# Lymphatus/caesium-clt

Hardware: AMD Instinct MI355X
Metric: megapixels/sec JPEG q=80 1920x1080 batch (higher is better)
Workload: dtype int32

## Files before the change

caesium-clt_amd/binding.py:

```python
import ctypes as C
import os

_HERE = os.path.dirname(os.path.abspath(__file__))
NPHASES = 8
NKERNELS = 36
PHASE_NAMES = ["decode", "pixel", "masks_flags_runs", "stats_tables", "sizes_scan", "pack", "stuff_assemble", "reserved"]


class CCSParameters(C.Structure):
    _fields_ = [("keep_metadata", C.c_bool), ("jpeg_quality", C.c_uint32), ("jpeg_chroma_subsampling", C.c_uint32),
                ("jpeg_progressive", C.c_bool), ("jpeg_optimize", C.c_bool), ("jpeg_preserve_icc", C.c_bool),
                ("png_quality", C.c_uint32), ("png_optimization_level", C.c_uint32), ("png_force_zopfli", C.c_bool),
                ("png_optimize", C.c_bool), ("gif_quality", C.c_uint32), ("webp_quality", C.c_uint32), ("webp_lossless", C.c_bool),
                ("tiff_compression", C.c_uint32), ("tiff_deflate_level", C.c_uint32), ("width", C.c_uint32), ("height", C.c_uint32)]


class CCSResult(C.Structure):
    _fields_ = [("success", C.c_bool), ("code", C.c_uint32), ("error_message", C.c_char_p)]


class CByteArray(C.Structure):
    _fields_ = [("data", C.POINTER(C.c_uint8)), ("length", C.c_size_t)]


class Timing(C.Structure):
    _fields_ = [("total_ms", C.c_float), ("phase_ms", C.c_float * NPHASES), ("kernel_ms", C.c_float * NKERNELS), ("in_bytes", C.c_uint64), ("out_bytes", C.c_uint64),
                ("pixels", C.c_uint64), ("coef_bytes", C.c_uint64), ("n_images", C.c_uint32), ("n_failed", C.c_uint32), ("n_seq_decoded", C.c_uint32), ("n_par_fallback", C.c_uint32), ("n_par_short", C.c_uint32), ("n_prog_decoded", C.c_uint32), ("n_refine_chains", C.c_uint32), ("n_search_extra", C.c_uint32), ("n_fused_lists", C.c_uint32), ("n_list_refine", C.c_uint32), ("n_ac_in_lists", C.c_uint32), ("n_list_runs", C.c_uint32)]


class PngTiming(C.Structure):
    _fields_ = [("total_ms", C.c_float), ("kernel_ms", C.c_float * 16), ("in_bytes", C.c_uint64), ("out_bytes", C.c_uint64), ("pixels", C.c_uint64),
                ("raw_bytes", C.c_uint64), ("n_images", C.c_uint32), ("n_failed", C.c_uint32), ("n_trials", C.c_uint32)]


class CaesiumError(RuntimeError):
    def __init__(self, code, message):
        super().__init__(f"[{code}] {message}")
        self.code = code


def library_path():
    return os.path.join(_HERE, "libcaesium_hip.so")
# ... 412 lines not shown
```

caesium-clt_amd/csrc/batch.hpp:

```cpp
#pragma once
#include <array>
#include <chrono>
#include <map>
#include <string>
#include <vector>

#include "../../include/caesium_hip.h"
#include "devmem.hpp"
#include "jpeg_host.hpp"
#include "kernels.h"
#include "webp_kernels.h"

namespace csh {

struct Item {
    int code = 0;
    std::string msg;
    JpegInfo in;
    JpegInfo out;
    int image = -1;
    size_t file_size = 0;
    std::vector<uint8_t> meta_out;
};

// ... 59 lines not shown
    int cand_work[64]; int ncand;
    int Al_luma = 0, Al_chroma = 0;
    uint64_t best_luma = 0, best_chroma = 0;
    int split_luma = 0, split_chroma = 0;
    bool luma_on = false, chroma_on = false;
};

struct EncodePlan {
    std::vector<EncScan> script;
    std::vector<ScanWork> swork;
    uint32_t nslots = 0, nlist_slots = 0, ntok_slots = 0;
    uint32_t nref_slots = 0;
    uint32_t last_run_refine = 0;
    uint32_t list_run = CSH_LIST_RUN;
    uint32_t nlist_runs = 0, nref_runs = 0;
    uint32_t last_run_list_runs = 0;
    uint64_t total_corr = 0;
    uint64_t total_units = 0, total_words = 0;
    uint32_t max_units = 0;
    int ntables = 0;
    std::vector<TokPlan> plans;
    std::vector<int> plan_comp, plan_image;
    std::vector<EChunk> echunks;
    uint64_t tok_cap = 0;
    uint32_t tok_scale = 1;
    std::vector<TokRegion> regions;
    std::vector<uint32_t> region_est;
    uint32_t hist_rows = 0;
    std::vector<NzList> nzlists;
    std::vector<NzSet> nzsets;
// ... 152 lines not shown
    for (int i = 0; i < int(sizeof kKernelSlots / sizeof kKernelSlots[0]); i++) if (kKernelSlots[i].slot != i) return false;
    return true;
}
static_assert(sizeof kKernelSlots / sizeof kKernelSlots[0] == CSH_NKERNELS && int(KS_COUNT) == int(CSH_NKERNELS), "one row per csh_timing.kernel_ms slot");
static_assert(kernel_slots_in_order(), "row i of kKernelSlots describes slot i");

struct PlanSwitches {
    std::string profile;
    bool nz_once = true;
    bool tr_sort = true;
    int prog_par = -1;
    bool fused_420 = true;
    bool nz_fused = true;
    bool ref_list = true;
    uint32_t list_run = CSH_LIST_RUN;
    bool ac_tiles = false;
    static PlanSwitches read();
};

struct Laps {
    const bool trace;
    std::chrono::steady_clock::time_point at = std::chrono::steady_clock::now();
    std::string text;
    Laps();
    void lap(const char *what);
};

struct BatchPlanner {
    csh_batch *const b;
    const CByteArray *const inputs;
// ... 53 lines not shown
```

caesium-clt_amd/csrc/batch_plan.cpp:

```cpp
#include <algorithm>
#include <atomic>
#include <cmath>
#include <thread>

#include "batch.hpp"
#include "resize_host.h"

namespace csh {

static void build_dev_huff(const HuffSpec &h, DevHuff &d) {
    memset(&d, 0, sizeof d);
    for (int l = 0; l < 18; l++) d.maxcode[l] = -1;
    if (!h.present) return;
    int code = 0, p = 0;
    for (int l = 1; l <= 16; l++) {
        if (h.bits[l]) {
            d.valptr[l] = p - code;
            for (int i = 0; i < h.bits[l]; i++, p++, code++)
                if (l <= 9) {
                    int base = code << (9 - l);
                    for (int k = 0; k < (1 << (9 - l)); k++) d.look[(base + k) & 511] = uint16_t((l << 8) | h.vals[p]);
                }
            d.maxcode[l] = code - 1;
        }
// ... 179 lines not shown
        b->enc.nzlists[i].base = at; b->enc.nzlists[i].cap = uint32_t(cap);
        at += (cap + 3) & ~uint64_t(3);
    }
    b->enc.nz_cap = at + 64;
}

PlanSwitches PlanSwitches::read() {
    auto is = [](const char *name, const char *v) { const char *e = getenv(name); return e && !strcmp(e, v); };
    PlanSwitches s;
    const char *penv = getenv("CSH_PROFILE");
    s.profile = penv && *penv ? penv : "mozjpeg";
    s.nz_once = !is("CSH_NZ_ONCE", "0");
    s.tr_sort = !is("CSH_TR_SORT", "0");
    s.nz_fused = !is("CSH_NZ_FUSED", "0");
    s.ac_tiles = is("CSH_AC_TILES", "1");
    s.ref_list = is("CSH_REF_LIST", "1") || (s.ref_list && !is("CSH_REF_LIST", "0"));
    const char *pp = getenv("CSH_PROG_PAR");
    s.prog_par = pp && !strcmp(pp, "0") ? 0 : (pp && !strcmp(pp, "1") ? 1 : -1);
    s.fused_420 = !getenv("CSH_NO_FUSED_420");
    if (const char *lr = getenv("CSH_LIST_RUN")) { if (*lr) s.list_run = uint32_t(std::min(32, std::max(1, atoi(lr)))); }
    return s;
}

Laps::Laps() : trace(getenv("CSH_TRACE") != nullptr) {}
void Laps::lap(const char *what) {
    if (!trace) return;
    const auto now = std::chrono::steady_clock::now();
    char buf[64];
    snprintf(buf, sizeof buf, " %s %.1f", what, std::chrono::duration<double, std::milli>(now - at).count());
    text += buf; at = now;
}

BatchPlanner::BatchPlanner(csh_batch *b_, const CByteArray *inputs_, size_t count_, const CCSParameters *p_, const csp_pixels *px_)
    : b(b_), inputs(inputs_), count(count_), p(p_), px(px_), sw(PlanSwitches::read()), progressive(p_->jpeg_progressive) {}

void BatchPlanner::begin() {
    b->items.resize(count);
    quality_table(int(p->jpeg_quality), qout_nat);
    DevQuant qo; make_quant(qout_nat, qo);
    b->quants.push_back(qo);
    b->q_base = int(b->quants.size()) - 1;
    for (int q = 1; q <= 100; q++) { uint16_t tq[64]; quality_table(q, tq); DevQuant dq; make_quant(tq, dq); b->quants.push_back(dq); }
    b->progressive = progressive;
    b->enc.list_run = sw.list_run;

    add_script(b->enc.script, 3, true);
    add_script(b->enc.script, 1, true);
    add_script(b->enc.script, 3, false);
    add_script(b->enc.script, 1, false);
    script_base3 = progressive ? 0 : 16; script_base1 = progressive ? 10 : 17;
    const bool webp = b->webp, rgb_out = b->rgb_out;
    const std::string &profile = sw.profile;
    b->enc.search = progressive && !webp && !rgb_out && profile != "plain";
    const bool lossy_jpeg = !b->lossless && !webp && !rgb_out;
    b->tr.trellis = lossy_jpeg && (profile == "mozjpeg" || profile == "mozjpeg-trellis");
    b->tr.dering = lossy_jpeg && (profile == "mozjpeg" || profile == "mozjpeg-dering");
    b->tr.nz_once = b->tr.trellis && progressive && sw.nz_once && sw.tr_sort;
}

// ... 842 lines not shown
```

caesium-clt_amd/csrc/batch_run.cpp:

```cpp
#include <algorithm>

#include "batch.hpp"

namespace csh {
namespace {

class KernelMarks {
    hipEvent_t ev[CSH_NKERNELS + 1];
    int created = 0, next = 0;
    const hipStream_t st;

public:
    explicit KernelMarks(hipStream_t s) : st(s) {}
    KernelMarks(const KernelMarks &) = delete;
    KernelMarks &operator=(const KernelMarks &) = delete;
    ~KernelMarks() { for (int i = 0; i < created; i++) (void)hipEventDestroy(ev[i]); }
    int start() {
        for (; created <= CSH_NKERNELS; created++) CSH_CHECK(hipEventCreate(&ev[created]));
        CSH_CHECK(hipEventRecord(ev[0], st));
        return 0;
    }
    int claim(KernelSlot slot, hipEvent_t *e) {
        if (int(slot) != next || next >= CSH_NKERNELS) {
            csh_set_error("internal: timing mark '%s' out of order (slot %d is next)", slot < KS_COUNT ? kKernelSlots[slot].name : "?", next);
// ... 217 lines not shown

    int encode_begin() {
        fill_enc_ctx();
        launch_reset_works(st, b->enc.d_swork.p, c.nwork);
        if (!fused && (b->enc.d_nz_cursor.zero(st) || b->enc.d_nz_chunk_cnt.zero(st))) return -1;
        if (b->enc.d_symbits.zero(st) || b->enc.d_eobbits.zero(st) || (!eobrun_cleared && b->enc.d_eobrun.zero(st)) || b->enc.d_tables.zero(st) || b->enc.d_tok_cursor.zero(st) || b->enc.d_slot_eobh.zero(st) || b->enc.d_scan_pad.zero(st)) return -1;
#ifdef CSH_EMUL
        if (b->enc.d_raw.zero(st)) return -1;
#else
        if ((c.debug & 8192u) && b->enc.d_raw.zero(st)) return -1;
#endif
        MARK(KS_MEMSET_ENC);
        return 0;
    }

    void count_list_runs(const Stage &sg, bool gate) {
        for (uint32_t wi = sg.work0; (sg.nlr || sg.nrr) && wi < sg.work0 + sg.nwork; wi++) {
            const ScanWork &w = b->enc.swork[wi];
            if ((w.lr_base != 0xFFFFFFFFu || w.rr_base != 0xFFFFFFFFu) && (!gate || b->enc.work_active[wi])) b->enc.last_run_list_runs += ((w.nunits + 255u) / 256u + b->enc.list_run - 1u) / b->enc.list_run;
        }
    }

    void set_stage(const Stage &sg) {
        c.echunks = b->enc.d_echunks.p + sg.ech0; c.nechunks = sg.nech; c.slot0 = sg.slot0; c.nslots = sg.nslots;
        c.nzchunks = (fused ? b->enc.d_nzchunks_fused.p : b->enc.d_nzchunks.p) + sg.nzc0; c.nnzchunks = sg.nnzc;
        c.nz_build = sg.nz_build[fused ? 1 : 0]; c.nz_filter = sg.nz_filter[fused ? 1 : 0];
        c.list_slots = b->enc.d_list_slots.p + sg.ls0; c.nlist_slots = sg.nls; c.tok_slots = b->enc.d_tok_slots.p + sg.ts0; c.ntok_slots = sg.nts;
        c.ref_slots = b->enc.d_ref_slots.p + sg.rs0; c.nref_slots = sg.nrs;
        c.list_runs = b->enc.d_list_runs.p + sg.lr0; c.nlist_runs = sg.nlr; c.ref_runs = b->enc.d_ref_runs.p + sg.rr0; c.nref_runs = sg.nrr; c.list_run = b->enc.list_run;
    }

    int trellis() {
        const Stage &tg = b->tr.tstage;
        set_stage(tg);
        c.stats_only = 1;
        if (b->enc.d_long_cnt.zero(st)) return -1;
        c.nz_blk_cnt = b->tr.t_sort ? b->tr.d_tblk_cnt.p : nullptr;
        c.nz_blk_off = (b->tr.t_sort && b->tr.nz_once) ? b->tr.d_tblk_off.p : nullptr;
        launch_nzlist(st, c);
        c.nz_blk_cnt = nullptr; c.nz_blk_off = nullptr;
        if (b->tr.t_sort) {
            TrellisCtx ts;
            memset(&ts, 0, sizeof ts);
            ts.work = b->tr.d_twork.p; ts.nwork = int(b->tr.twork.size()); ts.blk_cnt = b->tr.d_tblk_cnt.p; ts.perm = b->tr.d_tperm.p;
            launch_trellis_sort(st, ts);
        }
        launch_tokens(st, c);
        launch_list_stats(st, c);
        count_list_runs(tg, false);
        launch_ac_runs(st, c);
        launch_gen_tables(st, b->enc.d_tables.p + tg.table0, int(tg.ntables));
        c.stats_only = 0;
        if (b->enc.d_nz_cursor.zero(st)) return -1;
        MARK(KS_TRELLIS_STATS);
        TrellisCtx tc;
        fill_trellis_ctx(tc);
        if (b->tr.d_tqueue.zero(st)) return -1;
        launch_trellis_ac(st, tc);
        MARK(KS_TRELLIS_AC);
        launch_trellis_dc(st, tc);
        launch_fix_dummy(st, b->d_imgs.p, nimg, b->max_dummy, b->d_coef.p);
        MARK(KS_TRELLIS_DC);
        return 0;
    }

    int stage(const Stage &sg, bool mark, bool gate) {
#define SMARK(slot) do { if (mark) MARK(slot); } while (0)
        set_stage(sg);
        c.work_active = gate ? b->enc.d_work_active.p : nullptr;
        a.work0 = int(sg.work0); a.nwork_run = int(sg.nwork);
        if (b->enc.d_long_cnt.zero(st)) return -1;
        launch_nzlist(st, c);
        SMARK(KS_NZLIST);
        launch_list_refine(st, c);
        for (uint32_t wi = sg.work0; sg.nrs && wi < sg.work0 + sg.nwork; wi++)
            if (b->enc.swork[wi].rs_base != 0xFFFFFFFFu && (!gate || b->enc.work_active[wi])) b->enc.last_run_refine++;
        count_list_runs(sg, gate);
        launch_tokens(st, c);
        SMARK(KS_TOKENS);
        launch_list_stats(st, c);
        SMARK(KS_LIST_STATS);
        launch_ac_runs(st, c);
        SMARK(KS_AC_RUNS);
        launch_gen_tables(st, b->enc.d_tables.p + sg.table0, int(sg.ntables));
        SMARK(KS_GEN_TABLES);
        launch_chunk_sizes(st, c);
        SMARK(KS_CHUNK_SIZES);
        launch_exclusive_scan(st, b->enc.d_chunk_bits.p + sg.slot0, b->enc.d_chunk_off.p + sg.slot0, sg.nslots, b->enc.d_scan_tmp.p, b->enc.d_scan_tmp.n);
        SMARK(KS_SCAN_CHUNK_BITS);
        launch_scan_sizes(st, a);
        launch_exclusive_scan(st, b->enc.d_scan_pad.p, b->enc.d_scan_raw_off.p, uint64_t(a.nwork), b->enc.d_scan_tmp.p, b->enc.d_scan_tmp.n);
        launch_scan_place(st, a);
// ... 72 lines not shown
        if (b->out.d_img_size.zero(st)) return -1;
        csw::launch_webp_yuv(st, b->wp.d_wimgs.p, nwimg, b->wp.wmax_luma, b->pix.d_rgb.p, b->wp.d_wwork.p);
        MARK(KS_WEBP_YUV);
        hipEvent_t mid;
        if (marks.claim(KS_WEBP_ENCODE, &mid)) return -1;
        if (csw::launch_webp_encode(st, b->wp.wimgs.data(), nwimg, b->wp.d_wimgs.p, b->wp.d_wwork.p, b->wp.d_wlevels.p, b->wp.d_wscratch.p, b->wp.d_wpart.p, b->out.d_out.p, b->out.d_img_size.p, b->out.d_status.p, mid)) return -1;
        MARK(KS_WEBP_ASSEMBLE);
        return finish(false);
    }
};

}

int run_once(csh_batch *b, csh_timing *t, bool requant_only) {
    Run r(b, t);
    b->enc.last_run_list_runs = 0;
    b->enc.last_run_fused = 0; b->enc.last_run_refine = 0; b->enc.last_run_ac_lists = 0;
    if (r.pools() || r.marks.start()) return -1;
    const bool from_pixels = requant_only && b->tr.dering;
    if (requant_only && !from_pixels) {
        if (r.requant()) return -1;
    } else {
        if (from_pixels ? r.skip_decode() : r.decode()) return -1;
        if (r.planes()) return -1;
        if (b->webp) return r.webp();
        if (b->rgb_out) return (r.marks.mark(KS_XFORM_DIRECT) || r.finish(false)) ? -1 : 0;
        if (r.pixels()) return -1;
    }
    if (r.encode_begin()) return -1;
    b->enc.last_run_fused = r.fused ? b->enc.n_fused : 0u;
    b->enc.last_run_ac_lists = r.fused ? b->enc.n_ac_lists : 0u;
// ... 9 lines not shown
```

caesium-clt_amd/csrc/k_aclist.hip:

```cpp
#include "kernels.h"
#include "wave.h"

namespace csh {

#define CSH_LP_WORDS 1024

__device__ __forceinline__ static uint32_t lbitlen(uint32_t v) { return 32u - uint32_t(__clz(v)); }
__device__ __forceinline__ static int lwave() { return int(threadIdx.x) / CSP_WAVE_THREADS; }

#define CSH_NZ_HALF 16
__device__ __forceinline__ static uint4 nz_load(const EncCtx &c, const NzSet &S, uint32_t u, int bx, int by, uint32_t oct) {
    uint4 q; q.x = q.y = q.z = q.w = 0u;
    if (u < S.nunits) {
        const int b = by * S.bw + bx;
        q = *reinterpret_cast<const uint4 *>(c.coef + (size_t(S.tile_base) + size_t(b >> 6)) * CSH_TILE_I16 + size_t((b & 63) * CSH_BLK_STRIDE) + size_t(oct) * CSH_OCT_STRIDE);
    }
    return q;
}
__device__ __forceinline__ static uint32_t nz_mask8(const uint4 &q, uint32_t oct) {
    uint32_t m = 0;
    m |= (q.x & 0xFFFFu) ? 1u : 0u;   m |= (q.x >> 16) ? 2u : 0u;
    m |= (q.y & 0xFFFFu) ? 4u : 0u;   m |= (q.y >> 16) ? 8u : 0u;
    m |= (q.z & 0xFFFFu) ? 16u : 0u;  m |= (q.z >> 16) ? 32u : 0u;
    m |= (q.w & 0xFFFFu) ? 64u : 0u;  m |= (q.w >> 16) ? 128u : 0u;
// ... 375 lines not shown
    uint16_t *eobrun = s_eob[wv];
    LFOR(l) {
        for (int i = l; i < 256; i += 64) lut[i] = c.tables[r.table_base].lut[i];
        uint4 zero; zero.x = zero.y = zero.z = zero.w = 0u;
        for (int i = 4 * l; i < CSH_LP_WORDS; i += 256) *reinterpret_cast<uint4 *>(buf + i) = zero;
    }
    CSP_WAVE_SYNC();
    uint32_t *out = c.raw + (raw_bit0 >> 5);
    uint64_t pos = raw_bit0 & 31u;
    uint32_t ww = 0;
    bool first_flush = true;
    const uint32_t Ss = r.Ss, Se = r.Se;
    const uint32_t zrl = lut[0xF0], zc = zrl & 0xFFFFu, zl = zrl >> 16;
    LV<uint32_t> x0, x1, x2, x3;
    bool ahead = false;
    for (uint32_t ci = 0; ci < nrun; ci++) {
        const ListSlot ls = nx;
        const bool more = ci + 1u < nrun;
        if (more) nx = list_chunk(c, lbase, r.nzrec + ci + 1u);
#ifdef CSH_EMUL
        {
            const uint64_t want = (raw_bit0 & 31u) + (c.chunk_off[cs0 + ci] - c.chunk_off[cs0]);
            if (c.overflow[1] ? pos > want : pos != want) { fprintf(stderr, "k_list_pack: chunk %u of a run does not start where the one before it ended\n", ci); abort(); }
        }
#endif
        CSP_WAVE_SYNC();
        {
            const uint32_t u0 = r.unit0 + 256u * ci, left = r.nunits_work - 256u * (r.j + ci), nun = left < 256u ? left : 256u;
            LFOR(l) for (int i = l; i < 256; i += 64) eobrun[i] = uint32_t(i) < nun ? c.eobrun[u0 + uint32_t(i)] : uint16_t(0);
        }
        CSP_WAVE_SYNC();
        if (!ahead) LFOR(l) list_load4(ls, 4u * uint32_t(l), x0[l], x1[l], x2[l], x3[l]);
        ahead = false;
        uint32_t carry = CSH_NZ_END;
        const uint32_t cpad = more ? 0u : pad;
        const uint32_t n_ext = ls.n + (cpad ? 1u : 0u);
        for (uint32_t g0 = 0; g0 < n_ext; g0 += 256) {
            const LV<uint32_t> e0 = x0, e1 = x1, e2 = x2, e3 = x3;
            if (g0 + 256u < n_ext) LFOR(l) list_load4(ls, g0 + 256u + 4u * uint32_t(l), x0[l], x1[l], x2[l], x3[l]);
            else if (more) { LFOR(l) list_load4(nx, 4u * uint32_t(l), x0[l], x1[l], x2[l], x3[l]); ahead = true; }
            const LV<uint32_t> p0 = lprev(e3, carry);
            carry = llast(e3);
            LV<uint32_t> v0, v1, v2, v3, n0, n1, n2, n3, z, len;
            LFOR(l) {
// ... 324 lines not shown
```

caesium-clt_amd/csrc/k_entropy.hip:

```cpp
#include "kernels.h"
#include "wave.h"

namespace csh {

#define CSH_PK_WORDS 1024

__device__ __forceinline__ static uint64_t band_mask(int Ss, int Se) { return (~0ull >> (63 - Se)) & (~0ull << Ss); }
__device__ __forceinline__ static int msb64(uint64_t v) { return 63 - __clzll(v); }
__device__ __forceinline__ static int bitlen32(unsigned v) { return 32 - __clz(v); }
__device__ __forceinline__ static int lane_id() { return int(threadIdx.x & 63); }

__device__ __forceinline__ static int unit_block(const CompGeom &g, uint32_t u) {
    int by = int(u) / g.real_bw, bx = int(u) - by * g.real_bw;
    return by * g.bw + bx;
}
__device__ __forceinline__ static bool get_bit(const uint64_t *w, uint32_t i) { return (w[i >> 6] >> (i & 63)) & 1; }

#ifndef CSH_EMUL
template <class Op>
__device__ __forceinline__ static uint32_t wave_scan_dpp(uint32_t v, Op op) {
    v = op(v, uint32_t(__builtin_amdgcn_update_dpp(0, int(v), 0x111, 0xf, 0xf, false)));
    v = op(v, uint32_t(__builtin_amdgcn_update_dpp(0, int(v), 0x112, 0xf, 0xf, false)));
    v = op(v, uint32_t(__builtin_amdgcn_update_dpp(0, int(v), 0x114, 0xf, 0xf, false)));
    v = op(v, uint32_t(__builtin_amdgcn_update_dpp(0, int(v), 0x118, 0xf, 0xf, false)));
// ... 478 lines not shown
__device__ static bool eob_run_end(const uint64_t *sym, uint32_t nunits, uint32_t u, uint32_t max_words, uint32_t &t) {
    t = nunits - 1;
    uint32_t i = u + 1;
    const uint32_t nwords = (nunits + 63) >> 6;
    for (uint32_t n = 0; i < nunits; n++) {
        if (n == max_words) return false;
        uint32_t wi = i >> 6;
        uint64_t bits = sym[wi] & (~0ull << (i & 63));
        if (bits) { uint32_t p = (wi << 6) + uint32_t(__ffsll((unsigned long long)bits) - 1); if (p < nunits) t = p - 1; return true; }
        i = (wi + 1) << 6;
        if (wi + 1 >= nwords) break;
    }
    return true;
}
#define CSH_LONG_RUN_WORDS 8
__global__ void __launch_bounds__(256) k_ac_runs(EncCtx c) {
    const int lane = lane_id();
    const uint32_t cs = c.slot0 + blockIdx.x * 4u + (threadIdx.x >> 6);
    if (cs >= c.slot0 + c.nslots) return;
    const SlotRec r = c.slots[cs];
    if (!(r.flags & 1u)) return;
    if (c.work_active && !c.work_active[r.work]) return;
    const uint32_t nunits = r.nunits_work;
    uint32_t *freq = c.tables[r.table_base].freq;
    const uint64_t *sym = c.sym_bits + r.word_base, *eob = c.eob_bits + r.word_base;
    uint32_t mine = 0;
    (void)mine; (void)lane;
    CSH_UNROLL
    for (int i = 0; i < 4; i++) {
        const uint32_t u = r.j * 256u + uint32_t(i) * 64u + uint32_t(lane);
        int my_nb = -1;
// ... 35 lines not shown
            const uint64_t m = __ballot(my_nb == nb);
            if (lane == nb) mine += uint32_t(__popcll(m));
        }
        if (__ballot(my_nb >= 4)) {
            for (int nb = 4; nb < 15; nb++) {
                const uint64_t m = __ballot(my_nb == nb);
                if (lane == nb) mine += uint32_t(__popcll(m));
            }
        }
#endif
    }
#ifndef CSH_EMUL
    if (mine && lane < 15) { atomicAdd(&freq[lane << 4], mine); atomicAdd(&c.slot_eobh[cs * 16u + uint32_t(lane)], mine); }
#endif
}
__global__ void __launch_bounds__(64) k_ac_runs_long(EncCtx c) {
    const uint32_t n = *c.long_cnt;
    for (uint32_t e = blockIdx.x; e < n; e += gridDim.x) {
        const ScanWork w = c.work[c.long_runs[2 * e]];
        const EncScan &sc = c.script[w.scan];
        const uint32_t u = c.long_runs[2 * e + 1];
        const uint64_t *sym = c.sym_bits + w.word_base;
        uint32_t *freq = c.tables[w.table_base].freq;
        auto count = [&](uint32_t run, uint32_t owner) {
            const int nb = bitlen32(run) - 1;
            atomicAdd(&freq[nb << 4], 1u); atomicAdd(&c.slot_eobh[size_t(w.first_chunk + (owner >> 8)) * 16u + uint32_t(nb)], 1u);
        };
#ifdef CSH_EMUL
        uint32_t t;
        eob_run_end(sym, w.nunits, u, 0xFFFFFFFFu, t);
// ... 433 lines not shown
    if (cs >= c.slot0 + c.nslots) return;
    const SlotRec r = c.slots[cs];
    const ScanWork &w = c.work[r.work];
    if (w.no_room || (c.work_active && !c.work_active[r.work])) return;
    const uint64_t scan0 = c.chunk_off[r.first_chunk];
    const uint64_t bit0 = w.raw_off * 8 + (c.chunk_off[cs] - scan0);
    const uint64_t nbits = c.chunk_bits[cs];
    c.raw[bit0 >> 5] = 0;
    const uint64_t lo = nbits ? (bit0 + nbits - 1) >> 5 : bit0 >> 5, hi = (bit0 + nbits + (r.j == r.nch - 1 ? 8 : 0)) >> 5;
    for (uint64_t wi = lo; wi <= hi; wi++) c.raw[wi] = 0;
}
void launch_zero_edges(hipStream_t st, const EncCtx &c) { if (c.nslots) CSH_LAUNCH(k_zero_edges, dim3((c.nslots + 255) / 256), dim3(256), st, c); }
void launch_tokens(hipStream_t st, const EncCtx &c) { if (c.nechunks) CSH_LAUNCH_PHASED(k_tokens, 6, dim3(c.nechunks), dim3(256), st, c); }
void launch_ac_runs(hipStream_t st, const EncCtx &c) {
    if (!c.nslots) return;
    CSH_LAUNCH(k_ac_runs, dim3((c.nslots + 3) / 4), dim3(256), st, c);
#ifdef CSH_EMUL
    CSH_LAUNCH(k_ac_runs_long, dim3(64), dim3(1), st, c);
#else
    CSH_LAUNCH(k_ac_runs_long, dim3(4096), dim3(64), st, c);
#endif
}
void launch_chunk_sizes(hipStream_t st, const EncCtx &c) { if (c.nslots) CSH_LAUNCH(k_chunk_sizes, dim3((c.nslots + 3) / 4), dim3(256), st, c); }
void launch_pack(hipStream_t st, const EncCtx &c) { if (c.ntok_slots) CSH_LAUNCH(k_pack, dim3((c.ntok_slots + 3) / 4), dim3(256), st, c); }

}
```

caesium-clt_amd/csrc/kernels.h:

```cpp
#pragma once
#include "gpu_rt.h"
#include "types.h"

namespace csh {

__host__ __device__ static inline int coef_off(int k) { return (k >> 3) * CSH_OCT_STRIDE + (k & 7); }
__host__ __device__ static inline size_t coef_index(uint32_t tile_base, int b, int k) {
    return (size_t(tile_base) + size_t(b >> 6)) * CSH_TILE_I16 + size_t((b & 63) * CSH_BLK_STRIDE) + size_t(coef_off(k));
}

#define CSH_RAW_OCT 8
__host__ __device__ static inline size_t raw_index(uint32_t tile_base, int b) { return size_t(tile_base) * CSH_TILE_I16 + size_t(b) * 64; }

__device__ __forceinline__ static int csh_plane_at(const uint8_t *p, int pitch, int cw, int ch, int y, int x) {
    y = y < 0 ? 0 : (y > ch - 1 ? ch - 1 : y);
    x = x < 0 ? 0 : (x > cw - 1 ? cw - 1 : x);
    return p[size_t(y) * pitch + x];
}
__device__ __forceinline__ static int csh_upsample_at(const uint8_t *p, int pitch, int cw, int ch, UpDesc u, int r, int xx) {
    switch (u.cls) {
    case CSH_UP_COPY: return csh_plane_at(p, pitch, cw, ch, r, xx);
    case CSH_UP_H2V1: {
        const int cx = xx >> 1, nb = (xx & 1) ? cx + 1 : cx - 1;
        return (3 * csh_plane_at(p, pitch, cw, ch, r, cx) + csh_plane_at(p, pitch, cw, ch, r, nb) + ((xx & 1) ? 2 : 1)) >> 2;
// ... 113 lines not shown
    uint32_t *nz_chunk_off;
    uint32_t *nz_chunk_cnt;
    uint8_t *nz_blk_cnt;
    uint16_t *nz_blk_off;
    const uint32_t *list_slots;
    uint32_t nlist_slots;
    const uint32_t *tok_slots;
    uint32_t ntok_slots;
    const uint32_t *ref_slots;
    uint32_t nref_slots;
    const uint32_t *list_runs;
    uint32_t nlist_runs;
    const uint32_t *ref_runs;
    uint32_t nref_runs;
    uint32_t list_run;
    uint32_t nz_build, nz_filter;
};
enum : uint32_t { TK_SYM = 0u, TK_RAW = 1u, TK_ACF = 2u, TK_REF = 3u, TK_EOB = 4u };
void launch_tokens(hipStream_t st, const EncCtx &c);
void launch_ac_runs(hipStream_t st, const EncCtx &c);
void launch_gen_tables(hipStream_t st, DevEncTable *tables, int ntables);
void launch_chunk_sizes(hipStream_t st, const EncCtx &c);
void launch_zero_edges(hipStream_t st, const EncCtx &c);
void launch_pack(hipStream_t st, const EncCtx &c);
void launch_nzlist(hipStream_t st, const EncCtx &c);
void launch_list_stats(hipStream_t st, const EncCtx &c);
void launch_list_refine(hipStream_t st, const EncCtx &c);
void launch_list_pack(hipStream_t st, const EncCtx &c);
void launch_nz_to_tiles(hipStream_t st, const NzSet *nzsets, const NzList *nzlists, const uint32_t *nz_pool, const uint32_t *nz_chunk_off, const uint32_t *nz_chunk_cnt,
                        uint32_t set, uint32_t nchunks, int16_t *coef);
// ... 84 lines not shown
```

caesium-clt_amd/csrc/pipeline.cpp:

```cpp
#include <algorithm>
#include <atomic>
#include <cmath>
#include <cstdarg>
#include <memory>
#include <thread>

#include "batch.hpp"
#include "../../include/vp8_tables.h"
#include "resize_host.h"

static thread_local char g_err[512];
void csh_set_error(const char *fmt, ...) {
    va_list ap;
    va_start(ap, fmt);
    vsnprintf(g_err, sizeof g_err, fmt, ap);
    va_end(ap);
}
extern "C" const char *csh_last_error(void) { return g_err; }

#ifdef CSH_EMUL
thread_local dim3 threadIdx, blockIdx, blockDim, gridDim;
int csh_emul_reverse = 0;
thread_local int csh_emul_phase = 0;
extern "C" void csh_emul_set_reverse(int r) { csh_emul_reverse = r; }
// ... 211 lines not shown
            std::vector<uint32_t> rc(b->dec.d_relax_cnt.n);
            if (csh_copy_wait(rc.data(), b->dec.d_relax_cnt.p, rc.size() * sizeof(uint32_t), hipMemcpyDeviceToHost, b->stream) == hipSuccess) {
                fprintf(stderr, "[csh] relax list sizes (of %u sub-sequences):", b->dec.total_sub);
                for (size_t i = 0; i < rc.size() && (i < 16 || rc[i]); i++) fprintf(stderr, " %u", rc[i]);
                fprintf(stderr, "\n");
            }
        }
        for (const ProgChain &pc : b->dec.chains) if (pc.refine && ns[size_t(pc.image)] == 4) t->n_refine_chains++;
        for (uint32_t v : ns) { if (v == 4) { t->n_prog_decoded++; continue; } if (v) t->n_seq_decoded++; if (v == 2 || v == 3) t->n_par_fallback++; if (v == 3) t->n_par_short++; }
        t->n_images = uint32_t(b->nimg);
        t->n_search_extra = b->enc.search ? b->enc.n_gated_runs : 0u;
        t->n_fused_lists = b->enc.last_run_fused;
        t->n_list_refine = b->enc.last_run_refine;
        t->n_ac_in_lists = b->enc.last_run_ac_lists;
        t->n_list_runs = b->enc.last_run_list_runs;
        for (const Item &it : b->items) if (it.image < 0) t->n_failed++;
        for (int i = 0; i < b->nimg; i++) { t->out_bytes += b->out.h_img_size[i]; t->pixels += uint64_t(b->imgs[i].width) * b->imgs[i].height; }
        t->in_bytes = b->dec.bits_pool.size();
        uint64_t in_tiles = 0;
        for (const ImgDesc &im : b->imgs) for (int c = 0; c < im.ncomp; c++) in_tiles += im.in[c].ntiles;
        t->coef_bytes = in_tiles * CSH_TILE_I16 * 2;
    }
    b->out.ran = true;
    if (!requant_only) b->have_dct = (b->retain_dct || b->tr.trellis) && !b->lossless;
    return 0;
}

static void set_result(CCSResult *r, int code, const std::string &msg) {
    r->success = code == 0;
    r->code = uint32_t(code);
// ... 85 lines not shown
```

include/caesium_hip.h:

```cpp
#ifndef CAESIUM_HIP_H
#define CAESIUM_HIP_H
#include <stdbool.h>
#include <stddef.h>
#include <stdint.h>
#ifdef __cplusplus
extern "C" {
#endif

enum { CS_TYPE_JPEG = 0, CS_TYPE_PNG = 1, CS_TYPE_GIF = 2, CS_TYPE_WEBP = 3, CS_TYPE_TIFF = 4, CS_TYPE_UNKN = 5 };

enum {
    CS_OK = 0,
    CS_ERR_NO_DEVICE = 10001,
    CS_ERR_UNKNOWN_TYPE = 10200,
    CS_ERR_UNSUPPORTED = 10201,
    CS_ERR_BAD_JPEG = 20100,
    CS_ERR_JPEG_FEATURE = 20101,
    CS_ERR_POOL_OVERFLOW = 20200,
    CS_ERR_BAD_PNG = 30100,
    CS_ERR_BAD_WEBP = 40100,
    CS_ERR_SAME_FORMAT = 10407,
    CS_ERR_TOO_BIG = 10500
};

// ... 55 lines not shown
    float kernel_ms[CSH_NKERNELS];
    uint64_t in_bytes, out_bytes;
    uint64_t pixels;
    uint64_t coef_bytes;
    uint32_t n_images, n_failed;
    uint32_t n_seq_decoded;
    uint32_t n_par_fallback;
    uint32_t n_par_short;
    uint32_t n_prog_decoded;
    uint32_t n_refine_chains;
    uint32_t n_search_extra;
    uint32_t n_fused_lists;
    uint32_t n_list_refine;
    uint32_t n_ac_in_lists;
    uint32_t n_list_runs;
} csh_timing;

int csh_device_count(void);
const char *csh_last_error(void);
void csh_warmup(int device);
void csh_release_cached_memory(void);
const char *csh_kernel_name(int slot);
const char *csh_kernel_name_webp(int slot);
int csh_batch_create(const CByteArray *inputs, size_t count, const CCSParameters *p, int device, csh_batch **out);
int csh_batch_create_webp(const CByteArray *inputs, size_t count, const CCSParameters *p, int device, csh_batch **out);
int csh_batch_create_pixels(const CByteArray *inputs, size_t count, const CCSParameters *p, int device, csh_batch **out);
int csh_batch_pixels(csh_batch *b, size_t image, const uint8_t **device_pixels, uint32_t *width, uint32_t *height, uint32_t *channels, const char **message);
struct csp_pixels_s;
int csh_batch_create_from_pixels(const struct csp_pixels_s *sources, size_t count, const CCSParameters *p, int device, csh_batch **out);
int csh_batch_run(csh_batch *b, csh_timing *t);
// ... 58 lines not shown
```

Before: 44500.

## Compute EOB run lengths and histograms from per-word bitmasks in parallel

Replaces the per-slot EOB-run kernel with a word-parallel version: each thread handles one 64-unit word of the symbol and EOB bitmasks, derives run starts and short run lengths with bit tricks and popcounts, and reduces histogram counts across the wave with DPP and readlane before doing atomics. The AC list kernel also rebuilds short EOB runs inline from the same bitmasks instead of loading eobrun from memory, with a prefetch of the next chunk's words. The aim is to cut serial per-run work, global loads and atomic traffic in the progressive AC path. In exchange it adds considerable bit-manipulation complexity and a fallback path for long runs. It is on by default and can be disabled with CSH_EOB_WORDS=0.

```diff
diff --git a/caesium-clt_amd/binding.py b/caesium-clt_amd/binding.py
--- a/caesium-clt_amd/binding.py
+++ b/caesium-clt_amd/binding.py
@@ -25,7 +25,7 @@
 
 class Timing(C.Structure):
     _fields_ = [("total_ms", C.c_float), ("phase_ms", C.c_float * NPHASES), ("kernel_ms", C.c_float * NKERNELS), ("in_bytes", C.c_uint64), ("out_bytes", C.c_uint64),
-                ("pixels", C.c_uint64), ("coef_bytes", C.c_uint64), ("n_images", C.c_uint32), ("n_failed", C.c_uint32), ("n_seq_decoded", C.c_uint32), ("n_par_fallback", C.c_uint32), ("n_par_short", C.c_uint32), ("n_prog_decoded", C.c_uint32), ("n_refine_chains", C.c_uint32), ("n_search_extra", C.c_uint32), ("n_fused_lists", C.c_uint32), ("n_list_refine", C.c_uint32), ("n_ac_in_lists", C.c_uint32), ("n_list_runs", C.c_uint32)]
+                ("pixels", C.c_uint64), ("coef_bytes", C.c_uint64), ("n_images", C.c_uint32), ("n_failed", C.c_uint32), ("n_seq_decoded", C.c_uint32), ("n_par_fallback", C.c_uint32), ("n_par_short", C.c_uint32), ("n_prog_decoded", C.c_uint32), ("n_refine_chains", C.c_uint32), ("n_search_extra", C.c_uint32), ("n_fused_lists", C.c_uint32), ("n_list_refine", C.c_uint32), ("n_ac_in_lists", C.c_uint32), ("n_list_runs", C.c_uint32), ("n_eob_inline", C.c_uint32)]
 
 
 class PngTiming(C.Structure):
diff --git a/caesium-clt_amd/csrc/batch.hpp b/caesium-clt_amd/csrc/batch.hpp
--- a/caesium-clt_amd/csrc/batch.hpp
+++ b/caesium-clt_amd/csrc/batch.hpp
@@ -97,6 +97,8 @@
     uint32_t last_run_refine = 0;
     uint32_t list_run = CSH_LIST_RUN;
     uint32_t nlist_runs = 0, nref_runs = 0;
+    uint32_t eob_words = 1;
+    uint32_t last_run_eob_inline = 0;
     uint32_t last_run_list_runs = 0;
     uint64_t total_corr = 0;
     uint64_t total_units = 0, total_words = 0;
@@ -279,6 +281,7 @@
     bool nz_fused = true;
     bool ref_list = true;
     uint32_t list_run = CSH_LIST_RUN;
+    bool eob_words = true;
     bool ac_tiles = false;
     static PlanSwitches read();
 };
diff --git a/caesium-clt_amd/csrc/batch_plan.cpp b/caesium-clt_amd/csrc/batch_plan.cpp
--- a/caesium-clt_amd/csrc/batch_plan.cpp
+++ b/caesium-clt_amd/csrc/batch_plan.cpp
@@ -217,6 +217,7 @@
     s.tr_sort = !is("CSH_TR_SORT", "0");
     s.nz_fused = !is("CSH_NZ_FUSED", "0");
     s.ac_tiles = is("CSH_AC_TILES", "1");
+    s.eob_words = !is("CSH_EOB_WORDS", "0");
     s.ref_list = is("CSH_REF_LIST", "1") || (s.ref_list && !is("CSH_REF_LIST", "0"));
     const char *pp = getenv("CSH_PROG_PAR");
     s.prog_par = pp && !strcmp(pp, "0") ? 0 : (pp && !strcmp(pp, "1") ? 1 : -1);
@@ -246,6 +247,7 @@
     for (int q = 1; q <= 100; q++) { uint16_t tq[64]; quality_table(q, tq); DevQuant dq; make_quant(tq, dq); b->quants.push_back(dq); }
     b->progressive = progressive;
     b->enc.list_run = sw.list_run;
+    b->enc.eob_words = sw.eob_words ? 1u : 0u;
 
     add_script(b->enc.script, 3, true);
     add_script(b->enc.script, 1, true);
diff --git a/caesium-clt_amd/csrc/batch_run.cpp b/caesium-clt_amd/csrc/batch_run.cpp
--- a/caesium-clt_amd/csrc/batch_run.cpp
+++ b/caesium-clt_amd/csrc/batch_run.cpp
@@ -255,10 +255,13 @@
         return 0;
     }
 
-    void count_list_runs(const Stage &sg, bool gate) {
+    void count_list_runs(const Stage &sg, bool gate, bool packed) {
         for (uint32_t wi = sg.work0; (sg.nlr || sg.nrr) && wi < sg.work0 + sg.nwork; wi++) {
             const ScanWork &w = b->enc.swork[wi];
-            if ((w.lr_base != 0xFFFFFFFFu || w.rr_base != 0xFFFFFFFFu) && (!gate || b->enc.work_active[wi])) b->enc.last_run_list_runs += ((w.nunits + 255u) / 256u + b->enc.list_run - 1u) / b->enc.list_run;
+            if ((w.lr_base != 0xFFFFFFFFu || w.rr_base != 0xFFFFFFFFu) && (!gate || b->enc.work_active[wi])) {
+                b->enc.last_run_list_runs += ((w.nunits + 255u) / 256u + b->enc.list_run - 1u) / b->enc.list_run;
+                if (packed && b->enc.eob_words && w.lr_base != 0xFFFFFFFFu) b->enc.last_run_eob_inline++;
+            }
         }
     }
 
@@ -269,6 +272,7 @@
         c.list_slots = b->enc.d_list_slots.p + sg.ls0; c.nlist_slots = sg.nls; c.tok_slots = b->enc.d_tok_slots.p + sg.ts0; c.ntok_slots = sg.nts;
         c.ref_slots = b->enc.d_ref_slots.p + sg.rs0; c.nref_slots = sg.nrs;
         c.list_runs = b->enc.d_list_runs.p + sg.lr0; c.nlist_runs = sg.nlr; c.ref_runs = b->enc.d_ref_runs.p + sg.rr0; c.nref_runs = sg.nrr; c.list_run = b->enc.list_run;
+        c.eob_words = b->enc.eob_words;
     }
 
     int trellis() {
@@ -288,7 +292,7 @@
         }
         launch_tokens(st, c);
         launch_list_stats(st, c);
-        count_list_runs(tg, false);
+        count_list_runs(tg, false, false);
         launch_ac_runs(st, c);
         launch_gen_tables(st, b->enc.d_tables.p + tg.table0, int(tg.ntables));
         c.stats_only = 0;
@@ -316,7 +320,7 @@
         launch_list_refine(st, c);
         for (uint32_t wi = sg.work0; sg.nrs && wi < sg.work0 + sg.nwork; wi++)
             if (b->enc.swork[wi].rs_base != 0xFFFFFFFFu && (!gate || b->enc.work_active[wi])) b->enc.last_run_refine++;
-        count_list_runs(sg, gate);
+        count_list_runs(sg, gate, true);
         launch_tokens(st, c);
         SMARK(KS_TOKENS);
         launch_list_stats(st, c);
@@ -419,7 +423,7 @@
 
 int run_once(csh_batch *b, csh_timing *t, bool requant_only) {
     Run r(b, t);
-    b->enc.last_run_list_runs = 0;
+    b->enc.last_run_list_runs = 0; b->enc.last_run_eob_inline = 0;
     b->enc.last_run_fused = 0; b->enc.last_run_refine = 0; b->enc.last_run_ac_lists = 0;
     if (r.pools() || r.marks.start()) return -1;
     const bool from_pixels = requant_only && b->tr.dering;
diff --git a/caesium-clt_amd/csrc/eob_words.h b/caesium-clt_amd/csrc/eob_words.h
--- /dev/null
+++ b/caesium-clt_amd/csrc/eob_words.h
@@ -0,0 +1,64 @@
+#pragma once
+#include "gpu_rt.h"
+
+namespace csh {
+
+struct EobWord { uint64_t s, s1, start, near; };
+
+__device__ __forceinline__ static EobWord eob_word(uint64_t s, uint64_t s1, uint64_t e, uint32_t prev, uint32_t b0, uint32_t nunits) {
+    const uint32_t n_in = nunits - b0;
+    const uint64_t vm = n_in >= 64u ? ~0ull : ((1ull << n_in) - 1ull);
+    EobWord m;
+    m.s = s | ~vm;
+    m.s1 = n_in <= 64u ? ~0ull : (n_in >= 128u ? s1 : (s1 | (~0ull << (n_in - 64u))));
+    e &= vm;
+    const uint64_t pe = (e << 1) | uint64_t(b0 == 0u ? 0u : (prev & 1u));
+    m.start = e & (m.s | ~pe);
+    m.near = m.s1 ? m.start : (m.s ? (m.start & ((1ull << (63 - __clzll((unsigned long long)m.s))) - 1ull)) : 0ull);
+    return m;
+}
+__device__ __forceinline__ static uint32_t eob_word_len(const EobWord &m, uint32_t bit) {
+    const uint64_t hi = bit == 63u ? 0ull : (m.s >> (bit + 1u));
+    if (hi) return uint32_t(__ffsll((unsigned long long)hi));
+    return 63u - bit + uint32_t(__ffsll((unsigned long long)m.s1));
+}
+struct EobChunkWords { uint64_t s[5], e[4]; uint32_t prev; };
+__device__ __forceinline__ static EobChunkWords eob_chunk_words(const uint64_t *sym, const uint64_t *eob, uint32_t w0, uint32_t nwords) {
+    EobChunkWords cw;
+    CSH_UNROLL
+    for (uint32_t k = 0; k < 5; k++) cw.s[k] = sym[w0 + k < nwords ? w0 + k : nwords - 1u];
+    CSH_UNROLL
+    for (uint32_t k = 0; k < 4; k++) cw.e[k] = eob[w0 + k < nwords ? w0 + k : nwords - 1u];
+    cw.prev = uint32_t(eob[w0 ? w0 - 1u : 0u] >> 63);
+    return cw;
+}
+struct EobPair { uint64_t lo, hi; };
+__device__ __forceinline__ static EobPair eob_shr_and(EobPair a, EobPair b, uint32_t k) {
+    EobPair r;
+    r.lo = a.lo & ((b.lo >> k) | (b.hi << (64u - k)));
+    r.hi = a.hi & (b.hi >> k);
+    return r;
+}
+__device__ __forceinline__ static uint64_t eob_word_counts(const EobWord &m) {
+    EobPair n; n.lo = ~m.s; n.hi = ~m.s1;
+    EobPair ones; ones.lo = ones.hi = ~0ull;
+    const EobPair w1 = eob_shr_and(ones, n, 1), w2 = eob_shr_and(w1, w1, 1), w3 = eob_shr_and(w1, w2, 1), w4 = eob_shr_and(w2, w2, 2), w7 = eob_shr_and(w3, w4, 3),
+                  w8 = eob_shr_and(w4, w4, 4), w15 = eob_shr_and(w7, w8, 7), w16 = eob_shr_and(w8, w8, 8), w31 = eob_shr_and(w15, w16, 15), w32 = eob_shr_and(w16, w16, 16),
+                  w63 = eob_shr_and(w31, w32, 31);
+    const uint64_t a = m.near;
+    return uint64_t(__popcll((unsigned long long)(a & ~w1.lo))) | (uint64_t(__popcll((unsigned long long)(a & w1.lo & ~w3.lo))) << 8) |
+           (uint64_t(__popcll((unsigned long long)(a & w3.lo & ~w7.lo))) << 16) | (uint64_t(__popcll((unsigned long long)(a & w7.lo & ~w15.lo))) << 24) |
+           (uint64_t(__popcll((unsigned long long)(a & w15.lo & ~w31.lo))) << 32) | (uint64_t(__popcll((unsigned long long)(a & w31.lo & ~w63.lo))) << 40) |
+           (uint64_t(__popcll((unsigned long long)(a & w63.lo))) << 48);
+}
+__device__ __forceinline__ static uint64_t eob_word_counts14(const EobWord &m, uint64_t &fast) {
+    EobPair n; n.lo = ~m.s; n.hi = ~m.s1;
+    EobPair ones; ones.lo = ones.hi = ~0ull;
+    const EobPair w1 = eob_shr_and(ones, n, 1), w2 = eob_shr_and(w1, w1, 1), w3 = eob_shr_and(w1, w2, 1), w4 = eob_shr_and(w2, w2, 2), w7 = eob_shr_and(w3, w4, 3),
+                  w14 = eob_shr_and(w7, w7, 7);
+    const uint64_t a = fast = m.near & ~w14.lo;
+    return uint64_t(__popcll((unsigned long long)(a & ~w1.lo))) | (uint64_t(__popcll((unsigned long long)(a & w1.lo & ~w3.lo))) << 8) |
+           (uint64_t(__popcll((unsigned long long)(a & w3.lo & ~w7.lo))) << 16) | (uint64_t(__popcll((unsigned long long)(a & w7.lo))) << 24);
+}
+
+}
diff --git a/caesium-clt_amd/csrc/k_aclist.hip b/caesium-clt_amd/csrc/k_aclist.hip
--- a/caesium-clt_amd/csrc/k_aclist.hip
+++ b/caesium-clt_amd/csrc/k_aclist.hip
@@ -1,5 +1,6 @@
 #include "kernels.h"
 #include "wave.h"
+#include "eob_words.h"
 
 namespace csh {
 
@@ -413,6 +414,8 @@
     const uint32_t zrl = lut[0xF0], zc = zrl & 0xFFFFu, zl = zrl >> 16;
     LV<uint32_t> x0, x1, x2, x3;
     bool ahead = false;
+    EobChunkWords cw_next = {};
+    if (c.eob_words) cw_next = eob_chunk_words(c.sym_bits + r.word_base, c.eob_bits + r.word_base, r.j * 4u, (r.nunits_work + 63u) >> 6);
     for (uint32_t ci = 0; ci < nrun; ci++) {
         const ListSlot ls = nx;
         const bool more = ci + 1u < nrun;
@@ -426,7 +429,27 @@
         CSP_WAVE_SYNC();
         {
             const uint32_t u0 = r.unit0 + 256u * ci, left = r.nunits_work - 256u * (r.j + ci), nun = left < 256u ? left : 256u;
-            LFOR(l) for (int i = l; i < 256; i += 64) eobrun[i] = uint32_t(i) < nun ? c.eobrun[u0 + uint32_t(i)] : uint16_t(0);
+            if (!c.eob_words) {
+                LFOR(l) for (int i = l; i < 256; i += 64) eobrun[i] = uint32_t(i) < nun ? c.eobrun[u0 + uint32_t(i)] : uint16_t(0);
+            } else {
+                const uint32_t w0 = (r.j + ci) * 4u, nwords = (r.nunits_work + 63u) >> 6;
+                const bool cuts = r.nunits_work >= 0x7FFFu;
+                const EobChunkWords cw = cw_next;
+                if (more) cw_next = eob_chunk_words(c.sym_bits + r.word_base, c.eob_bits + r.word_base, w0 + 4u, nwords);
+                CSH_UNROLL
+                for (uint32_t k = 0; k < 4; k++) {
+                    const uint32_t w = w0 + k;
+                    if (w >= nwords) { LFOR(l) eobrun[64u * k + uint32_t(l)] = uint16_t(0); continue; }
+                    const EobWord m = eob_word(cw.s[k], w + 1u < nwords ? cw.s[k + 1] : ~0ull, cw.e[k], k ? uint32_t(cw.e[k - 1] >> 63) : cw.prev, w * 64u, r.nunits_work);
+                    LFOR(l) {
+                        const uint32_t i = 64u * k + uint32_t(l);
+                        uint32_t run = 0;
+                        if ((m.near >> l) & 1) run = eob_word_len(m, uint32_t(l));
+                        else if ((((m.start >> l) & 1) || cuts) && i < nun) run = c.eobrun[u0 + i];
+                        eobrun[i] = uint16_t(run);
+                    }
+                }
+            }
         }
         CSP_WAVE_SYNC();
         if (!ahead) LFOR(l) list_load4(ls, 4u * uint32_t(l), x0[l], x1[l], x2[l], x3[l]);
diff --git a/caesium-clt_amd/csrc/k_entropy.hip b/caesium-clt_amd/csrc/k_entropy.hip
--- a/caesium-clt_amd/csrc/k_entropy.hip
+++ b/caesium-clt_amd/csrc/k_entropy.hip
@@ -1,5 +1,6 @@
 #include "kernels.h"
 #include "wave.h"
+#include "eob_words.h"
 
 namespace csh {
 
@@ -516,7 +517,7 @@
     return true;
 }
 #define CSH_LONG_RUN_WORDS 8
-__global__ void __launch_bounds__(256) k_ac_runs(EncCtx c) {
+__global__ void __launch_bounds__(256) k_ac_runs_slots(EncCtx c) {
     const int lane = lane_id();
     const uint32_t cs = c.slot0 + blockIdx.x * 4u + (threadIdx.x >> 6);
     if (cs >= c.slot0 + c.nslots) return;
@@ -582,6 +583,114 @@
     if (mine && lane < 15) { atomicAdd(&freq[lane << 4], mine); atomicAdd(&c.slot_eobh[cs * 16u + uint32_t(lane)], mine); }
 #endif
 }
+__device__ __forceinline__ static void ac_run_general(const EncCtx &c, const SlotRec &r, uint32_t u) {
+    const uint32_t nunits = r.nunits_work;
+    uint32_t *freq = c.tables[r.table_base].freq;
+    ScanWork w; w.unit_base = r.unit_base; w.word_base = r.word_base; w.nunits = nunits; w.first_chunk = r.first_chunk; w.table_base = r.table_base;
+    EncScan sc; sc.Ss = r.Ss; sc.Se = r.Se; sc.Ah = r.Ah; sc.Al = r.Al;
+    uint32_t t;
+    if (eob_run_end(c.sym_bits + r.word_base, nunits, u, CSH_LONG_RUN_WORDS, t))
+        eob_run_serial(c, w, sc, u, t, [&](uint32_t run, uint32_t owner) {
+            const int nb = bitlen32(run) - 1;
+            atomicAdd(&freq[nb << 4], 1u); atomicAdd(&c.slot_eobh[size_t(r.first_chunk + (owner >> 8)) * 16u + uint32_t(nb)], 1u);
+        });
+    else { uint32_t e = atomicAdd(c.long_cnt, 1u); c.long_runs[2 * e] = r.work; c.long_runs[2 * e + 1] = u; }
+}
+#ifndef CSH_EMUL
+__device__ __forceinline__ static uint32_t quad_sum(uint32_t v) {
+    v += uint32_t(__builtin_amdgcn_update_dpp(0, int(v), 0xB1 , 0xf, 0xf, false));
+    v += uint32_t(__builtin_amdgcn_update_dpp(0, int(v), 0x4E , 0xf, 0xf, false));
+    return v;
+}
+#endif
+__global__ void __launch_bounds__(256) k_ac_runs(EncCtx c) {
+    const uint32_t tid = blockIdx.x * 256u + threadIdx.x;
+    const uint32_t cs = c.slot0 + (tid >> 2), q = tid & 3u;
+    uint64_t cnt = 0;
+    bool slot_ok = false;
+    uint32_t table_base = 0xFFFFFFFFu;
+    uint64_t fast = 0, fs = 0, fs1 = 0;
+    uint32_t fbase = 0;
+    if (cs < c.slot0 + c.nslots) {
+        const SlotRec r = c.slots[cs];
+        slot_ok = (r.flags & 1u) && !(c.work_active && !c.work_active[r.work]);
+        const uint32_t nunits = r.nunits_work, b0 = r.j * 256u + q * 64u;
+        if (slot_ok) table_base = r.table_base;
+        if (slot_ok && b0 < nunits) {
+            const uint64_t *sym = c.sym_bits + r.word_base, *eob = c.eob_bits + r.word_base;
+            const uint32_t w0 = b0 >> 6, nwords = (nunits + 63) >> 6;
+            const uint64_t s = sym[w0], e = eob[w0];
+            const uint64_t s1 = w0 + 1 < nwords ? sym[w0 + 1] : ~0ull;
+            const uint32_t prev = w0 ? uint32_t(eob[w0 - 1] >> 63) : 0u;
+            const EobWord m = eob_word(s, s1, e, prev, b0, nunits);
+            const bool inl = r.Ah == 0 && ((r.flags & 4u) || c.stats_only);
+            uint64_t todo = m.start;
+            if (inl) { cnt = eob_word_counts(m); todo &= ~m.near; }
+            else if (r.Ah != 0) { cnt = eob_word_counts14(m, fast); todo &= ~fast; fs = m.s; fs1 = m.s1; fbase = r.unit_base + b0; }
+            while (todo) {
+                const uint32_t bit = uint32_t(__ffsll((unsigned long long)todo) - 1);
+                todo &= todo - 1;
+                const uint32_t u = b0 + bit;
+                const uint32_t len = ((m.near >> bit) & 1) ? eob_word_len(m, bit) : 0xFFFFFFFFu;
+                if (len <= 14u || (len < 0x7FFFu && r.Ah == 0)) {
+                    c.eobrun[r.unit_base + u] = uint16_t(len);
+                    cnt += 1ull << (8 * (bitlen32(len) - 1));
+                } else ac_run_general(c, r, u);
+            }
+        }
+    }
+#ifdef CSH_EMUL
+    for (uint64_t f = fast; f; f &= f - 1) {
+        const uint32_t bit = uint32_t(__ffsll((unsigned long long)f) - 1);
+        EobWord m; m.s = fs; m.s1 = fs1; m.start = m.near = fast;
+        c.eobrun[fbase + bit] = uint16_t(eob_word_len(m, bit));
+    }
+#else
+    for (uint64_t pend = __ballot(fast != 0); pend; pend &= pend - 1) {
+        const int src = __ffsll((unsigned long long)pend) - 1;
+        auto get64 = [&](uint64_t v) { return uint64_t(uint32_t(__builtin_amdgcn_readlane(int(uint32_t(v)), src))) | (uint64_t(uint32_t(__builtin_amdgcn_readlane(int(uint32_t(v >> 32)), src))) << 32); };
+        EobWord m; m.s = get64(fs); m.s1 = get64(fs1); m.start = m.near = get64(fast);
+        const uint32_t base = uint32_t(__builtin_amdgcn_readlane(int(fbase), src)), bit = threadIdx.x & 63u;
+        if ((m.near >> bit) & 1) c.eobrun[base + bit] = uint16_t(eob_word_len(m, bit));
+    }
+#endif
+#ifdef CSH_EMUL
+    if (slot_ok)
+        for (uint32_t nb = 0; nb < 7; nb++) {
+            const uint32_t n = uint32_t(cnt >> (8 * nb)) & 255u;
+            if (n) { atomicAdd(&c.tables[table_base].freq[nb << 4], n); atomicAdd(&c.slot_eobh[cs * 16u + nb], n); }
+        }
+#else
+    const uint64_t okm = __ballot(slot_ok);
+    if (!okm) return;
+    uint32_t p[4], qs[4];
+    CSH_UNROLL
+    for (int k = 0; k < 4; k++) {
+        p[k] = (uint32_t(cnt >> (16 * k)) & 255u) | ((uint32_t(cnt >> (16 * k + 8)) & 255u) << 16);
+        qs[k] = quad_sum(p[k]);
+    }
+    const uint32_t qa = (q & 1u ? (q & 2u ? qs[1] : qs[0]) >> 16 : (q & 2u ? qs[1] : qs[0])) & 0xFFFFu;
+    const uint32_t qb = q == 3u ? 0u : ((q & 1u ? (q & 2u ? qs[3] : qs[2]) >> 16 : (q & 2u ? qs[3] : qs[2])) & 0xFFFFu);
+    if (slot_ok) {
+        if (qa) atomicAdd(&c.slot_eobh[cs * 16u + q], qa);
+        if (qb) atomicAdd(&c.slot_eobh[cs * 16u + q + 4u], qb);
+    }
+    const uint32_t tb0 = uint32_t(__builtin_amdgcn_readlane(int(table_base), __ffsll((unsigned long long)okm) - 1));
+    if (__ballot(slot_ok && table_base != tb0) == 0) {
+        uint32_t t[4];
+        CSH_UNROLL
+        for (int k = 0; k < 4; k++) t[k] = uint32_t(__builtin_amdgcn_readlane(int(wave_incl_sum(p[k])), 63));
+        const uint32_t lane = threadIdx.x & 63u;
+        const uint32_t tw = lane & 4u ? (lane & 2u ? t[3] : t[2]) : (lane & 2u ? t[1] : t[0]);
+        const uint32_t n = (lane & 1u ? tw >> 16 : tw) & 0xFFFFu;
+        if (lane < 7u && n) atomicAdd(&c.tables[tb0].freq[lane << 4], n);
+    } else if (slot_ok) {
+        uint32_t *freq = c.tables[table_base].freq;
+        if (qa) atomicAdd(&freq[q << 4], qa);
+        if (qb) atomicAdd(&freq[(q + 4u) << 4], qb);
+    }
+#endif
+}
 __global__ void __launch_bounds__(64) k_ac_runs_long(EncCtx c) {
     const uint32_t n = *c.long_cnt;
     for (uint32_t e = blockIdx.x; e < n; e += gridDim.x) {
@@ -1045,7 +1154,8 @@
 void launch_tokens(hipStream_t st, const EncCtx &c) { if (c.nechunks) CSH_LAUNCH_PHASED(k_tokens, 6, dim3(c.nechunks), dim3(256), st, c); }
 void launch_ac_runs(hipStream_t st, const EncCtx &c) {
     if (!c.nslots) return;
-    CSH_LAUNCH(k_ac_runs, dim3((c.nslots + 3) / 4), dim3(256), st, c);
+    if (c.eob_words) CSH_LAUNCH(k_ac_runs, dim3((c.nslots + 63) / 64), dim3(256), st, c);
+    else CSH_LAUNCH(k_ac_runs_slots, dim3((c.nslots + 3) / 4), dim3(256), st, c);
 #ifdef CSH_EMUL
     CSH_LAUNCH(k_ac_runs_long, dim3(64), dim3(1), st, c);
 #else
diff --git a/caesium-clt_amd/csrc/kernels.h b/caesium-clt_amd/csrc/kernels.h
--- a/caesium-clt_amd/csrc/kernels.h
+++ b/caesium-clt_amd/csrc/kernels.h
@@ -151,6 +151,7 @@
     const uint32_t *ref_runs;
     uint32_t nref_runs;
     uint32_t list_run;
+    uint32_t eob_words;
     uint32_t nz_build, nz_filter;
 };
 enum : uint32_t { TK_SYM = 0u, TK_RAW = 1u, TK_ACF = 2u, TK_REF = 3u, TK_EOB = 4u };
diff --git a/caesium-clt_amd/csrc/pipeline.cpp b/caesium-clt_amd/csrc/pipeline.cpp
--- a/caesium-clt_amd/csrc/pipeline.cpp
+++ b/caesium-clt_amd/csrc/pipeline.cpp
@@ -249,6 +249,7 @@
         t->n_list_refine = b->enc.last_run_refine;
         t->n_ac_in_lists = b->enc.last_run_ac_lists;
         t->n_list_runs = b->enc.last_run_list_runs;
+        t->n_eob_inline = b->enc.last_run_eob_inline;
         for (const Item &it : b->items) if (it.image < 0) t->n_failed++;
         for (int i = 0; i < b->nimg; i++) { t->out_bytes += b->out.h_img_size[i]; t->pixels += uint64_t(b->imgs[i].width) * b->imgs[i].height; }
         t->in_bytes = b->dec.bits_pool.size();
diff --git a/include/caesium_hip.h b/include/caesium_hip.h
--- a/include/caesium_hip.h
+++ b/include/caesium_hip.h
@@ -93,6 +93,7 @@
     uint32_t n_list_refine;
     uint32_t n_ac_in_lists;
     uint32_t n_list_runs;
+    uint32_t n_eob_inline;
 } csh_timing;
 
 int csh_device_count(void);
```

Result: faster. 46190, median of 6 (+3.8%).
